# kouyt5/lightning-asr

Measured on AMD Instinct MI355X. Metric: audio-seconds/sec training (asr13x1, bs=32, 10 s clips), higher is better.
Workload: dtype bf16; 1 GPU; asr13x1 QuartzNet-CTC train step, bs=32/GPU, 10 s synthetic 16 kHz clips, labels.txt vocab (C=28), HIP mel+conv+CTC+NovoGrad, random-init weights; global_batch=32, n_class=28, parallelism=dp1, feature_prefetch=True, hip_graph=True, staged_backward=False

## Files before the change

lightning_asr_amd/csrc/conv.hip:

```cpp
#include "common.h"
#include "fused.h"

namespace lasr {

static thread_local const DwTapCtx* g_dw_tap_ctx = nullptr;
void dw_taps_set_ctx(const DwTapCtx* ctx) { g_dw_tap_ctx = ctx; }
bool dw_taps_enabled() {
  static const bool on = !(getenv("LASR_DW_TAPS") && atoi(getenv("LASR_DW_TAPS")) == 0);
  return on;
}
const uint32_t* dw_taps_for(const float* w, int flip, int64_t C) {
  (void)flip;
  const DwTapCtx* c = g_dw_tap_ctx;
  if (!c || C % 64 != 0) return nullptr;
  for (int i = 0; i < c->n; ++i)
    if (c->w[i] == w && c->C[i] == (int)C) return c->t[i];
  return nullptr;
}

static constexpr int kCB = 64;
static constexpr int kTT = 128;
static constexpr int kR = 8;
static constexpr int kMaxK = 128;

// ... 415 lines not shown
        o[0] += a[0]; o[1] += a[1]; o[2] += a[2]; o[3] += a[3];
      }
      Elem<bf16_t>::st4(y + off, o);
    }
  }
}

namespace dwm {
static constexpr int TT = 512;
static constexpr int KWMAX = 128;
static constexpr int TIN = TT - 16 + KWMAX;
static constexpr int LDI = 1296;
static constexpr int RS = 128;
static constexpr int LDST = 160;
static constexpr int IMG_BYTES = kCB * LDI;
static constexpr int STAGE_BYTES = RS * LDST;
static constexpr int WROW = 160;
static constexpr int WSM_OFF = IMG_BYTES + STAGE_BYTES;
static constexpr int SMEM = WSM_OFF + kCB * WROW * 4;
static_assert(LDI >= TIN * 2 && LDI % 16 == 0, "image pitch");
}
struct DwBnIn {
  const bf16_t* y; const bf16_t* y2; const float* coef; const float* coef2; bf16_t* out; int act;
};
typedef __bf16 dw_bf16x8 __attribute__((ext_vector_type(8)));
typedef float dw_f32x4 __attribute__((ext_vector_type(4)));
typedef short dw_s16x4 __attribute__((ext_vector_type(4)));

#ifdef LASR_DW_STAMPS
__device__ unsigned long long* g_dw_stamps = nullptr;
#define DW_STAMP(i_) do { if (g_dw_stamps && threadIdx.x == 0) g_dw_stamps[(blockIdx.y * gridDim.x + blockIdx.x) * 8 + (i_)] = wall_clock64(); } while (0)
#else
#define DW_STAMP(i_) do {} while (0)
#endif
template <int NKS, int NSET, bool FUSE = false>
__device__ __forceinline__ void dwconv_s1_mfma_body(const bf16_t* __restrict__ x, const float* __restrict__ w,
                                                    const bf16_t* __restrict__ addend, bf16_t* __restrict__ y,
                                                    int Tlen, int C, int k, int flip, int bx, int by, int bz, int gz,
                                                    char* smem_raw, const uint32_t* __restrict__ taps, const DwBnIn bn = DwBnIn{}) {
  using namespace dwm;
  char* img = smem_raw;
  char* stage = smem_raw + IMG_BYTES;
  uint32_t* wsm = reinterpret_cast<uint32_t*>(smem_raw + WSM_OFF);
  const int tid = threadIdx.x, lane = tid & 63, wid = tid >> 6;
  const int b = by, c0 = bx * kCB;
  if (taps) {
// ... 9 lines not shown
    float f0[kIt], f1[kIt];
#pragma unroll
    for (int it = 0; it < kIt; ++it) {
      const int i = tid + 512 * it;
      const int ch = i / WROW, idx = i - ch * WROW;
      const int i0 = idx < 80 ? 2 * idx : 2 * (idx - 80) + 1;
      const int j0 = i0 - 24, j1 = i0 - 23;
      const float* wc = w + (size_t)min(c0 + ch, C - 1) * k;
      const bool cok = c0 + ch < C;
      const int q0 = min(max(j0, 0), k - 1), q1 = min(max(j1, 0), k - 1);
      const float a0 = wc[flip ? k - 1 - q0 : q0], a1 = wc[flip ? k - 1 - q1 : q1];
      f0[it] = __uint_as_float(__float_as_uint(a0) & ((cok && j0 >= 0 && j0 < k) ? 0xffffffffu : 0u));
      f1[it] = __uint_as_float(__float_as_uint(a1) & ((cok && j1 >= 0 && j1 < k) ? 0xffffffffu : 0u));
    }
    __builtin_amdgcn_sched_barrier(0);
#pragma unroll
    for (int it = 0; it < kIt; ++it) wsm[tid + 512 * it] = (uint32_t)f32_to_bf16(f0[it]) | ((uint32_t)f32_to_bf16(f1[it]) << 16);
  }
  const int pad = k / 2, P = (pad + 7) & ~7, sh = P - pad;
  constexpr int KW = 32 * NKS;
  const bf16_t* xb = FUSE ? nullptr : x + (size_t)b * Tlen * C;
  const int n16 = lane & 15, g4 = lane >> 4;
  float ca[8], cb[8], ca2[8], cb2[8];
  if (FUSE) {
    const int ccl = min(c0 + ((tid & 7) << 3), C - 8);
    auto ld8 = [](const float* p, float (&o)[8]) {
      const float4 u = *reinterpret_cast<const float4*>(p), q = *reinterpret_cast<const float4*>(p + 4);
      o[0] = u.x; o[1] = u.y; o[2] = u.z; o[3] = u.w; o[4] = q.x; o[5] = q.y; o[6] = q.z; o[7] = q.w;
    };
    ld8(bn.coef + ccl, ca); ld8(bn.coef + C + ccl, cb);
    if (bn.y2) { ld8(bn.coef2 + ccl, ca2); ld8(bn.coef2 + C + ccl, cb2); }
  }

  DW_STAMP(0);
  constexpr int TTS = 256 * NSET;
  for (int tA = bz * TTS; tA < Tlen; tA += TTS * gz) {
    const int tin = TTS - 16 + KW;
    constexpr int kRounds = (TTS - 16 + KWMAX + RS - 1) / RS;
    uint4 v[kRounds][2];
    if (!FUSE) {
#pragma unroll
      for (int r = 0; r < kRounds; ++r) {
#pragma unroll
        for (int h = 0; h < 2; ++h) {
          const int ch = tid + 512 * h;
          const int tau = r * RS + (ch >> 3);
          const int t = tA - P + tau;
          const int cc = c0 + ((ch & 7) << 3);
          const bool ok = tau < tin && t >= 0 && t < Tlen && cc < C;
          const uint4 ld = *reinterpret_cast<const uint4*>(xb + (size_t)min(max(t, 0), Tlen - 1) * C + min(cc, C - 8));
          const uint32_t mk = ok ? 0xffffffffu : 0u;
          v[r][h] = make_uint4(ld.x & mk, ld.y & mk, ld.z & mk, ld.w & mk);
        }
      }
    } else {
      uint4 ly[kRounds][2], lr[kRounds][2];
      const size_t ub = (size_t)b * Tlen * C;
#pragma unroll
      for (int r = 0; r < kRounds; ++r) {
#pragma unroll
        for (int h = 0; h < 2; ++h) {
          const int ch = tid + 512 * h;
          const int t = tA - P + r * RS + (ch >> 3);
          const size_t off = ub + (size_t)min(max(t, 0), Tlen - 1) * C + min(c0 + ((ch & 7) << 3), C - 8);
          ly[r][h] = Vec<bf16_t>::raw(bn.y + off);
          if (bn.y2) lr[r][h] = Vec<bf16_t>::raw(bn.y2 + off);
        }
      }
      with_act(bn.act, [&](auto act_c) {
      constexpr int act = decltype(act_c)::value;
#pragma unroll
      for (int r = 0; r < kRounds; ++r) {
#pragma unroll
        for (int h = 0; h < 2; ++h) {
          const int ch = tid + 512 * h;
          const int tau = r * RS + (ch >> 3);
          const int t = tA - P + tau;
          const int cc = c0 + ((ch & 7) << 3);
          const bool ok = tau < tin && t >= 0 && t < Tlen && cc < C;
          float yv[8], rv[8], o[8];
          Vec<bf16_t>::unpack(ly[r][h], yv);
#pragma unroll
          for (int j = 0; j < 8; ++j) o[j] = fmaf(yv[j], ca[j], cb[j]);
          if (bn.y2) {
            Vec<bf16_t>::unpack(lr[r][h], rv);
#pragma unroll
            for (int j = 0; j < 8; ++j) o[j] += fmaf(rv[j], ca2[j], cb2[j]);
          }
#pragma unroll
          for (int j = 0; j < 8; ++j) o[j] = act_fwd(o[j], act);
          const uint4 pk = Vec<bf16_t>::pack(o);
// ... 822 lines not shown
        hipLaunchKernelGGL(dwconv_s1_bf16_kernel, grid, dim3(256), sh1, as_stream(stream), (const bf16_t*)x, w, (const bf16_t*)addend,
                           (bf16_t*)y, Tin, C, k, flip);
      }
    }
  } else {
    const bool small = (int64_t)grid.x * grid.y * grid.z < 200;
    const dim3 g2 = small ? dim3((unsigned)cdiv(Tout, 64), grid.y, grid.z) : grid;
#define LASR_DWF(T_, R_)                                                                                                          \
  do {                                                                                                                            \
    (void)hipFuncSetAttribute(reinterpret_cast<const void*>(dwconv_fwd_kernel<T_, R_>), hipFuncAttributeMaxDynamicSharedMemorySize, 160 * 1024); \
    hipLaunchKernelGGL((dwconv_fwd_kernel<T_, R_>), g2, dim3(256), shmem, as_stream(stream), (const T_*)x, w, (const T_*)addend, (T_*)y, Tin,  \
                       Tout, C, k, stride, flip);                                                                                 \
  } while (0)
    if (dtype == LASR_F32) { if (small) LASR_DWF(float, 4); else LASR_DWF(float, 8); }
    else { if (small) LASR_DWF(bf16_t, 4); else LASR_DWF(bf16_t, 8); }
#undef LASR_DWF
  }
  prof_end(tok, as_stream(stream));
  LASR_LAUNCH_CHECK("dwconv_fwd_kernel");
  return 0;
}

int lasr::dwconv_fwd_bn(const void* y, const float* coef, const void* y2, const float* coef2, int act, const float* w, void* out, void* u,
                        int64_t B, int64_t T, int64_t C, int k, void* stream) {
  LASR_CHECK_ARG(y && coef && w && out && u && (!y2 || coef2), "dwconv_fwd_bn: null pointer");
  static const bool off = getenv("LASR_DWCONV_FMA") || getenv("LASR_DWCONV_DOT2");
  const int padk = k / 2, shk = ((padk + 7) & ~7) - padk;
  auto al16 = [](const void* p) { return reinterpret_cast<uintptr_t>(p) % 16 == 0; };
  if (off || k < 1 || k > kMaxK || !(k & 1) || C % 8 != 0 || C < 8 || 15 + k + shk > dwm::KWMAX || T <= 0 || T >= (1 << 30) || B <= 0 ||
      B >= 65536 || !al16(y) || !al16(y2) || !al16(out) || !al16(u) || !al16(coef) || !al16(coef2))
    return 1;
  const int nks = (15 + k + shk + 31) / 32;
  static const bool no_half = getenv("LASR_DWCONV_NO_HALF") != nullptr;
  const bool half = !no_half && T > 256 && cdiv(C, kCB) * B * cdiv(T, (int64_t)512) < 200;
  static const bool full_too = getenv("LASR_BN_DW_FUSE") && atoi(getenv("LASR_BN_DW_FUSE")) == 2;
  if (!half && !full_too) return 1;
  const dim3 gridm((unsigned)cdiv(C, kCB), (unsigned)B, half ? (unsigned)std::min<int64_t>(cdiv(T, (int64_t)256), 8) : 1u);
  DwBnIn bn;
  bn.y = (const bf16_t*)y; bn.y2 = (const bf16_t*)y2; bn.coef = coef; bn.coef2 = coef2; bn.out = (bf16_t*)out; bn.act = act;
  const int tok = prof_begin(LASR_PROF_DWCONV, as_stream(stream), 2.0 * (double)B * T * C * k, (double)B * T * C * (y2 ? 4 : 3) * 2);
  const uint32_t* taps = dw_taps_for(w, 0, C);
#define LASR_DWMB2(N_, S_)                                                                                                  \
  do {                                                                                                                      \
    (void)hipFuncSetAttribute(reinterpret_cast<const void*>(dwconv_s1_mfma_bn_kernel<N_, S_>), hipFuncAttributeMaxDynamicSharedMemorySize, 160 * 1024); \
    hipLaunchKernelGGL((dwconv_s1_mfma_bn_kernel<N_, S_>), gridm, dim3(512), dwm::SMEM, as_stream(stream), bn, w, (bf16_t*)u, (int)T, (int)C, k, taps); \
  } while (0)
#define LASR_DWMB(N_) do { if (half) LASR_DWMB2(N_, 1); else LASR_DWMB2(N_, 2); } while (0)
  if (nks == 1) LASR_DWMB(1); else if (nks == 2) LASR_DWMB(2); else if (nks == 3) LASR_DWMB(3); else LASR_DWMB(4);
#undef LASR_DWMB
#undef LASR_DWMB2
  prof_end(tok, as_stream(stream));
  LASR_LAUNCH_CHECK("dwconv_s1_mfma_bn_kernel");
  return 0;
}

extern "C" size_t lasr_dwconv_wgrad_workspace_bytes(int64_t B, int64_t Tout, int64_t C, int k) {
  return (size_t)B * cdiv(Tout, kWChunkG) * C * k * sizeof(float);
}

static int dwconv_wgrad_impl(const void* x, const void* dy, float* dw, int dtype, int64_t B, int64_t Tin, int64_t C, int k,
                            int stride, void* workspace, size_t workspace_bytes, void* stream, int* n_partials_out);

// ... 170 lines not shown
```

lightning_asr_amd/csrc/fused.h:

```cpp
#pragma once
#include "common.h"

namespace lasr {

int dwconv_fwd_bn(const void* y, const float* coef, const void* y2, const float* coef2, int act, const float* w, void* out, void* u,
                  int64_t B, int64_t T, int64_t C, int k, void* stream);

static constexpr int kDwTapRow = 160;
struct DwTapJobs {
  int n; int blk0[17]; const float* w[16]; uint32_t* out[16]; int C[16]; int k[16];
};
__device__ __forceinline__ uint32_t dw_tap_entry(const float* __restrict__ w, int C, int k, int e) {
  const int flip = e / (C * kDwTapRow), r = e - flip * (C * kDwTapRow);
  const int c = r / kDwTapRow, idx = r - c * kDwTapRow;
  const int i0 = idx < kDwTapRow / 2 ? 2 * idx : 2 * (idx - kDwTapRow / 2) + 1;
  const int j0 = i0 - 24, j1 = i0 - 23;
  const float* wc = w + (size_t)c * k;
  const int q0 = min(max(j0, 0), k - 1), q1 = min(max(j1, 0), k - 1);
  const float a0 = wc[flip ? k - 1 - q0 : q0], a1 = wc[flip ? k - 1 - q1 : q1];
  const uint32_t m0 = (j0 >= 0 && j0 < k) ? 0xffffffffu : 0u, m1 = (j1 >= 0 && j1 < k) ? 0xffffffffu : 0u;
  return (uint32_t)f32_to_bf16(__uint_as_float(__float_as_uint(a0) & m0)) | ((uint32_t)f32_to_bf16(__uint_as_float(__float_as_uint(a1) & m1)) << 16);
}
struct DwTapCtx { int n; const float* w[16]; const uint32_t* t[16]; int C[16]; };
void dw_taps_set_ctx(const DwTapCtx* ctx);
const uint32_t* dw_taps_for(const float* w, int flip, int64_t C);
bool dw_taps_enabled();

int mask_lengths_step_cast(const float* pct, int64_t B, int64_t T_, int32_t* lens, uint64_t* step_counter, const float* in, void* out,
                           int64_t n, const DwTapJobs* jobs, void* stream);
// ... 12 lines not shown
```

lightning_asr_amd/csrc/model.hip:

```cpp
#include "common.h"
#include "mel.h"
#include "fused.h"
#include "gemm.h"
#include "lstm_body.h"
#include "se_seqsum.h"
#include <string>
#include <vector>
#include <math.h>

extern "C" size_t lasr_bn_bwd_workspace_bytes(int64_t B, int64_t T, int64_t C);
extern "C" size_t lasr_gemm_workspace_bytes(int64_t M, int64_t N, int split_k, int want_stats);
extern "C" size_t lasr_dwconv_wgrad_workspace_bytes(int64_t B, int64_t Tout, int64_t C, int k);
extern "C" int lasr_log_softmax_bwd(const float*, const float*, float*, int64_t, int64_t, void*);
extern "C" int lasr_cast_f32_to_bf16(const float*, void*, int64_t, void*);
extern "C" int lasr_colsum_f32(const float* x, float* out, int64_t rows, int64_t C, void* workspace, size_t workspace_bytes, void* stream);
extern "C" size_t lasr_colsum_workspace_bytes(int64_t rows, int64_t C);
extern "C" int lasr_scale_sum_f32(const float* x, int64_t n, float scale, float* out, void* stream);
extern "C" int lasr_seqsum(const void* x, int dtype, int64_t B, int64_t T, int64_t C, float* sums, void* stream);
extern "C" int lasr_se_fwd(const float* sums, const float* coef, const float* W1, const float* W2, int64_t B, int64_t T, int64_t C,
                           float* pooled, float* hidden, float* scale, void* stream);
extern "C" size_t lasr_se_bwd_workspace_bytes(int64_t B, int64_t C);
extern "C" int lasr_se_bwd(const void* dout, const void* y, const float* coef, const void* y2, const float* coef2, const float* scale,
                           const float* hidden, const float* pooled, const float* W1, const float* W2, int dtype, int64_t B, int64_t T,
                           int64_t C, int act, float* seg, float* dW1, float* dW2, void* workspace, size_t workspace_bytes, void* stream);
// ... 504 lines not shown
  if (!training) {
    std::vector<lasr_bn_eval_desc> descs;
    for (const Unit& u : m->units) {
      descs.push_back({params + u.bn.gamma, params + u.bn.beta, buffers + u.bn.rmean, buffers + u.bn.rvar, atf(ws, u.o_coef), u.co});
      if (u.has_res)
        descs.push_back({params + u.bn_res.gamma, params + u.bn_res.beta, buffers + u.bn_res.rmean, buffers + u.bn_res.rvar,
                         atf(ws, u.o_coef2), u.co});
    }
    for (size_t i = 0; i < descs.size(); i += 64)
      LASR_TRY(lasr_bn_eval_coef_many(descs.data() + i, (int)std::min<size_t>(64, descs.size() - i), kBnEps, stream));
    if (eval_fold(m->cfg.dtype)) {
      std::vector<lasr_fold_desc> fd;
      for (const Unit& u : m->units)
        if (fold_unit(u))
          fd.push_back({params + u.w_pw, params + u.w_res, atf(ws, u.o_coef), atf(ws, u.o_coef2), at(ws, u.o_wfold), atf(ws, u.o_bfold), u.co, u.ci});
      for (size_t i = 0; i < fd.size(); i += 32)
        LASR_TRY(lasr_fold_bn_weights_many(fd.data() + i, (int)std::min<size_t>(32, fd.size() - i), stream));
    }
  }
  const void* x = feats;
  int64_t Tx = T_in;
  static const bool bn_dw_fuse = !(getenv("LASR_BN_DW_FUSE") && atoi(getenv("LASR_BN_DW_FUSE")) == 0);
  const Unit* pend = nullptr;
  auto bn_act_of = [&](const Unit& v) -> int {
    ProfScope ps_bn(LASR_PROF_BN, stream, (double)N * v.co * dtype_size(dt) * (v.has_res ? 3 : 2));
    const lasr_dropout drop = {m->drop_step, m->drop_seed, (uint32_t)(&v - m->units.data()), dropping ? m->drop_p : 0.f};
    return lasr_bn_act_fwd_drop(at(ws, v.o_y), atf(ws, v.o_coef), v.has_res ? at(ws, v.o_y2) : nullptr,
                                v.has_res ? atf(ws, v.o_coef2) : nullptr, v.has_se ? atf(ws, v.o_se_scale) : nullptr, at(ws, v.o_out), dt, B,
                                T, v.co, v.act ? m->cfg.act : LASR_ACT_NONE, dropping ? &drop : nullptr, stream);
  };
  RoctxRange rr_fwd(training ? "lasr:forward (training)" : "lasr:forward (eval)");
  for (size_t ui = 0; ui < m->units.size(); ++ui) {
    const Unit& u = m->units[ui];
    RoctxRange rr_unit(u.rx_fwd.c_str());
    if (pend && !(u.has_dw && u.stride == 1 && !u.ctx_before)) {
      LASR_TRY(bn_act_of(*pend));
      pend = nullptr;
    }
    if (u.ctx_before) {
      {
        lasr_gemm_problem pr[2];
        for (int d = 0; d < 2; ++d) pr[d] = {x, wptr(m, params, ws, m->lstm.w_ih[d]), atf(ws, p.o_gx[d]), N, 160, 256, nullptr, nullptr, 0, nullptr};
        LASR_TRY(lasr_gemm_batch(pr, 2, dt, LASR_F32, 0, 0, 1, scratch, p.scratch_bytes, stream));
      }
      LASR_TRY(lasr_copy_cols(x, dt, 256, 0, at(ws, p.o_cat), dt, 336, 0, N, 256, 0, stream));
      LASR_TRY(lasr_bilstm_fwd(atf(ws, p.o_gx[0]), atf(ws, p.o_gx[1]), params + m->lstm.w_hh[0], params + m->lstm.w_hh[1],
                               params + m->lstm.b_ih[0], params + m->lstm.b_hh[0], params + m->lstm.b_ih[1], params + m->lstm.b_hh[1],
                               lens, B, T, at(ws, p.o_cat), dt, 336, 256, atf(ws, p.o_lstm_saved), stream));
      x = at(ws, p.o_cat);
    }
    const void* gin = x;
    if (u.has_dw) {
      int fused = 1;
      if (pend) {
        fused = dwconv_fwd_bn(at(ws, pend->o_y), atf(ws, pend->o_coef), pend->has_res ? at(ws, pend->o_y2) : nullptr,
                              pend->has_res ? atf(ws, pend->o_coef2) : nullptr, pend->act ? m->cfg.act : LASR_ACT_NONE, params + u.w_dw,
                              at(ws, pend->o_out), at(ws, u.o_u), B, T, u.ci, u.k, stream);
        if (fused < 0) return fused;
        if (fused == 1) LASR_TRY(bn_act_of(*pend));
        pend = nullptr;
      }
      if (fused == 1) LASR_TRY(lasr_dwconv_fwd(x, params + u.w_dw, nullptr, at(ws, u.o_u), dt, B, Tx, u.ci, u.k, u.stride, 0, stream));
      gin = at(ws, u.o_u);
    }
    if (!training && eval_fold(dt) && fold_unit(u)) {
      LASR_TRY(lasr_gemm_dual(gin, u.ci, x, u.ci, at(ws, u.o_wfold), atf(ws, u.o_bfold), at(ws, u.o_out), N, u.co, u.masked ? lens : nullptr,
                              T, u.act ? m->cfg.act : LASR_ACT_NONE, stream));
      x = at(ws, u.o_out);
      Tx = T;
      continue;
    }
    float* stats = training ? atf(ws, u.o_stats) : nullptr;
    float* stats2 = (training && u.has_res) ? atf(ws, u.o_stats2) : nullptr;
    bool se_sums_done = false;
    {
      lasr_gemm_problem pr[2];
      pr[0] = {gin, wptr(m, params, ws, u.w_pw), at(ws, u.o_y), N, u.co, u.ci, nullptr, u.masked ? lens : nullptr, T, stats};
      if (u.has_res) pr[1] = {x, wptr(m, params, ws, u.w_res), at(ws, u.o_y2), N, u.co, u.ci, nullptr, nullptr, 0, stats2};
      const int np = u.has_res ? 2 : 1;
      if (training && !no_fuse()) {
        const float* parts[2] = {nullptr, nullptr};
        int tiles[2] = {0, 0};
        LASR_TRY(lasr_gemm_batch_partials(pr, np, dt, dt, 0, 0, scratch, p.scratch_bytes, parts, tiles, stream));
        lasr_bn_branch br[2];
        br[0] = {parts[0], tiles[0], params + u.bn.gamma, params + u.bn.beta, buffers + u.bn.rmean, buffers + u.bn.rvar,
                 atf(ws, u.o_coef), atf(ws, u.o_saved), stats};
        if (u.has_res)
          br[1] = {parts[1], tiles[1], params + u.bn_res.gamma, params + u.bn_res.beta, buffers + u.bn_res.rmean,
                   buffers + u.bn_res.rvar, atf(ws, u.o_coef2), atf(ws, u.o_saved2), stats2};
        ProfScope ps(LASR_PROF_BN, stream, 0.0);
        int merged = 1;
        if (u.has_se) {
          merged = bn_finalize_partials_seqsum(br, np, u.co, N, kBnEps, kBnMom, at(ws, u.o_y), dt, B, T, atf(ws, u.o_se_sum), stream);
          if (merged < 0 || merged > 1) return merged;
          se_sums_done = merged == 0;
        }
        if (merged == 1) LASR_TRY(lasr_bn_finalize_partials(br, np, u.co, N, kBnEps, kBnMom, stream));
      } else {
        LASR_TRY(lasr_gemm_batch(pr, np, dt, dt, 0, 0, 1, scratch, p.scratch_bytes, stream));
        if (training) {
          LASR_TRY(lasr_bn_finalize(stats, params + u.bn.gamma, params + u.bn.beta, buffers + u.bn.rmean, buffers + u.bn.rvar,
                                    atf(ws, u.o_coef), atf(ws, u.o_saved), u.co, N, kBnEps, kBnMom, training, stream));
          if (u.has_res)
            LASR_TRY(lasr_bn_finalize(stats2, params + u.bn_res.gamma, params + u.bn_res.beta, buffers + u.bn_res.rmean,
                                      buffers + u.bn_res.rvar, atf(ws, u.o_coef2), atf(ws, u.o_saved2), u.co, N, kBnEps, kBnMom,
                                      training, stream));
        }
      }
    }
    bool se_applied = false;
    if (u.has_se) {
      ProfScope ps_se(LASR_PROF_BN, stream, (double)N * u.co * dtype_size(dt));
      if (!se_sums_done) LASR_TRY(lasr_seqsum(at(ws, u.o_y), dt, B, T, u.co, atf(ws, u.o_se_sum), stream));
      int folded = 1;
      if (training && !dropping && !no_fuse())
        folded = bn_se_act_fwd(at(ws, u.o_y), atf(ws, u.o_coef), u.has_res ? at(ws, u.o_y2) : nullptr, u.has_res ? atf(ws, u.o_coef2) : nullptr,
                               atf(ws, u.o_se_sum), params + u.w_se1, params + u.w_se2, at(ws, u.o_out), atf(ws, u.o_se_pool),
                               atf(ws, u.o_se_hid), atf(ws, u.o_se_scale), dt, B, T, u.co, u.act ? m->cfg.act : LASR_ACT_NONE, stream);
      if (folded < 0 || folded > 1) return folded;
      se_applied = folded == 0;
// ... 387 lines not shown
```

lightning_asr_amd/csrc/norm.hip:

```cpp
#include "common.h"
#include "reduce_body.h"
#include "se_seqsum.h"
#include "fused.h"
#include "dropout.h"
#include <algorithm>
#include <string.h>

namespace lasr {

template <typename T, bool TO_BTC>
__global__ __launch_bounds__(256) void transpose_kernel(const void* __restrict__ in_, void* __restrict__ out_,
                                                        int64_t C, int64_t Tt) {
  __shared__ float tile[32][33];
  const int b = blockIdx.z;
  const int64_t c0 = (int64_t)blockIdx.y * 32, t0 = (int64_t)blockIdx.x * 32;
  const int tx = threadIdx.x & 31, ty = threadIdx.x >> 5;
  if (TO_BTC) {
    const float* in = reinterpret_cast<const float*>(in_) + (int64_t)b * C * Tt;
    T* out = reinterpret_cast<T*>(out_) + (int64_t)b * C * Tt;
    for (int i = ty; i < 32; i += 8)
      if (c0 + i < C && t0 + tx < Tt) tile[i][tx] = in[(c0 + i) * Tt + t0 + tx];
    __syncthreads();
    for (int i = ty; i < 32; i += 8)
      if (t0 + i < Tt && c0 + tx < C) Elem<T>::st(out + (t0 + i) * C + c0 + tx, tile[tx][i]);
  } else {
    const T* in = reinterpret_cast<const T*>(in_) + (int64_t)b * C * Tt;
    float* out = reinterpret_cast<float*>(out_) + (int64_t)b * C * Tt;
// ... 21 lines not shown
    return;
  }
  if ((int)blockIdx.x >= cast_blocks) {
    const int tb = (int)blockIdx.x - cast_blocks;
    int l = 0;
    while (l + 1 < jobs.n && jobs.blk0[l + 1] <= tb) ++l;
    const int e = (tb - jobs.blk0[l]) * 256 + (int)threadIdx.x;
    if (e < 2 * jobs.C[l] * kDwTapRow) jobs.out[l][e] = dw_tap_entry(jobs.w[l], jobs.C[l], jobs.k[l], e);
    return;
  }
  const int64_t n4 = n >> 2;
  const int64_t stride = (int64_t)cast_blocks * 256;
  for (int64_t e = blockIdx.x * (int64_t)256 + threadIdx.x; e < n4; e += stride) {
    const float4 v = reinterpret_cast<const float4*>(in)[e];
    uint2 o;
    o.x = (uint32_t)f32_to_bf16(v.x) | ((uint32_t)f32_to_bf16(v.y) << 16);
    o.y = (uint32_t)f32_to_bf16(v.z) | ((uint32_t)f32_to_bf16(v.w) << 16);
    reinterpret_cast<uint2*>(out)[e] = o;
  }
  if (blockIdx.x == 0)
    for (int64_t e = (n4 << 2) + threadIdx.x; e < n; e += 256) out[e] = f32_to_bf16(in[e]);
}

__device__ __forceinline__ void bn_finalize_channel(float s, float q, int64_t c, const float* __restrict__ gamma,
                                                    const float* __restrict__ beta, float* __restrict__ rmean,
                                                    float* __restrict__ rvar, float* __restrict__ coef, float* __restrict__ saved,
                                                    int64_t C, float n, float eps, float momentum, int training) {
  float mean, var;
  if (training) {
    const double m = (double)s / n;
    double v = (double)q / n - m * m;
    if (v < 0) v = 0;
    mean = (float)m;
    var = (float)v;
    if (rmean) {
      rmean[c] = (1.f - momentum) * rmean[c] + momentum * mean;
      const float unbiased = n > 1.f ? (float)(v * (double)n / ((double)n - 1.0)) : var;
      rvar[c] = (1.f - momentum) * rvar[c] + momentum * unbiased;
    }
  } else {
    mean = rmean[c];
    var = rvar[c];
  }
  const float rstd = 1.0f / sqrtf(var + eps);
  const float a = gamma[c] * rstd;
  coef[c] = a;
  coef[C + c] = beta[c] - mean * a;
  if (saved) { saved[c] = mean; saved[C + c] = rstd; }
}

__global__ void bn_finalize_kernel(const float* __restrict__ stats, const float* __restrict__ gamma,
                                   const float* __restrict__ beta, float* __restrict__ rmean, float* __restrict__ rvar,
                                   float* __restrict__ coef, float* __restrict__ saved, int64_t C, float n, float eps,
                                   float momentum, int training) {
  const int64_t c = blockIdx.x * (int64_t)blockDim.x + threadIdx.x;
  if (c >= C) return;
  bn_finalize_channel(training ? stats[c] : 0.f, training ? stats[C + c] : 0.f, c, gamma, beta, rmean, rvar, coef, saved, C, n, eps,
                      momentum, training);
}

struct BnEvalMany { lasr_bn_eval_desc d[64]; };
__global__ __launch_bounds__(256) void bn_eval_coef_many_kernel(BnEvalMany a, float eps) {
  const lasr_bn_eval_desc q = a.d[blockIdx.y];
  const int64_t c = blockIdx.x * (int64_t)blockDim.x + threadIdx.x;
  if (c >= q.C) return;
  bn_finalize_channel(0.f, 0.f, c, q.gamma, q.beta, const_cast<float*>(q.running_mean), const_cast<float*>(q.running_var), q.coef, nullptr,
                      q.C, 1.f, eps, 0.f, 0);
}

template <int LANES = 8>
__device__ __forceinline__ double partial_lane_sum(const float* __restrict__ partials, int n_part, int64_t ncols, int64_t c, int pl) {
  double a0 = 0.0, a1 = 0.0, a2 = 0.0, a3 = 0.0;
  for (int p = pl; p < n_part; p += 16 * LANES) {
    float v[16];
#pragma unroll
    for (int i = 0; i < 16; ++i) {
      const int r = p + LANES * i;
      const float x = partials[(int64_t)min(r, n_part - 1) * ncols + c];
      v[i] = r < n_part ? x : 0.f;
    }
#pragma unroll
    for (int i = 0; i < 16; i += 4) {
      a0 += (double)v[i]; a1 += (double)v[i + 1]; a2 += (double)v[i + 2]; a3 += (double)v[i + 3];
    }
  }
  return (a0 + a1) + (a2 + a3);
}

__global__ __launch_bounds__(256) void reduce_partials_kernel(const float* __restrict__ partials, int n_part, int64_t ncols,
                                                              float* __restrict__ out0, int64_t split, float* __restrict__ out1) {
  __shared__ double s_acc[8][33];
  const int cl = threadIdx.x & 31, pl = threadIdx.x >> 5;
  const int64_t c = (int64_t)blockIdx.x * 32 + cl;
  s_acc[pl][cl] = c < ncols ? partial_lane_sum(partials, n_part, ncols, c, pl) : 0.0;
  __syncthreads();
  if (pl == 0 && c < ncols) {
    double s = 0.0;
#pragma unroll
    for (int i = 0; i < 8; ++i) s += s_acc[i][cl];
    if (c < split) out0[c] = (float)s;
    else if (out1) out1[c - split] = (float)s;
  }
}

struct BnBranch {
  const float* partials; int n_part;
  const float* gamma; const float* beta; float* rmean; float* rvar; float* coef; float* saved; float* stats;
};
struct BnBranch2 { BnBranch b[2]; };

__global__ __launch_bounds__(256) void bn_finalize_partials_kernel(BnBranch2 br, int64_t C, float n, float eps, float momentum) {
  __shared__ double s_acc[8][33];
  const BnBranch& b = blockIdx.y ? br.b[1] : br.b[0];
  const int cl = threadIdx.x & 31, pl = threadIdx.x >> 5;
  const int64_t c = (int64_t)blockIdx.x * 16 + (cl & 15);
  s_acc[pl][cl] = c < C ? partial_lane_sum(b.partials, b.n_part, 2 * C, (int64_t)(cl >> 4) * C + c, pl) : 0.0;
  __syncthreads();
  if (pl == 0 && cl < 16 && c < C) {
    double s = 0.0, q = 0.0;
#pragma unroll
    for (int i = 0; i < 8; ++i) { s += s_acc[i][cl]; q += s_acc[i][16 + cl]; }
    if (b.stats) { b.stats[c] = (float)s; b.stats[C + c] = (float)q; }
    bn_finalize_channel((float)s, (float)q, c, b.gamma, b.beta, b.rmean, b.rvar, b.coef, b.saved, C, n, eps, momentum, 1);
  }
}

template <typename T>
__global__ __launch_bounds__(256) void bn_finalize_seqsum_kernel(BnBranch2 br, int64_t C, float n, float eps, float momentum, int nfx, int nf,
                                                                 const T* __restrict__ x, int Tt, int gx, float* __restrict__ sums) {
  constexpr int RL = 256 / (64 / Vec<T>::kN);
  __shared__ double s_acc[8][33];
  __shared__ float s_red[RL][65];
// ... 147 lines not shown
      for (int j = 0; j < V; ++j) {
        o[j] = fmaf(v[j], a[j], b[j]);
        if (SE) o[j] *= sev[u][j];
      }
      float dsc[V];
      if (DROP) drop_scale<V>(drop, drop_step, off[u], dsc);
      if (DROP && HAS2) {
#pragma unroll
        for (int j = 0; j < V; ++j) o[j] *= dsc[j];
      }
      if (HAS2) {
        Vec<T>::unpack(rw[u], w);
        tab_vec(s_tab + 2 * C, c, C, a); tab_vec(s_tab + 3 * C, c, C, b);
#pragma unroll
        for (int j = 0; j < V; ++j) o[j] += fmaf(w[j], a[j], b[j]);
      }
#pragma unroll
      for (int j = 0; j < V; ++j) o[j] = act_fwd(o[j], act);
      if (DROP && !HAS2) {
#pragma unroll
        for (int j = 0; j < V; ++j) o[j] *= dsc[j];
      }
      if (it0 + 256 * u < n_items) Vec<T>::store(out + off[u], o);
    }
  }
  });
}

template <typename T, bool HAS2, bool SE, bool DROP>
__global__ __launch_bounds__(256, 2) void bn_bwd_stats_kernel(const T* __restrict__ dout, const T* __restrict__ y,
                                                              const float* __restrict__ coef, const float* __restrict__ saved,
                                                              const T* __restrict__ y2, const float* __restrict__ coef2,
                                                              const float* __restrict__ saved2, const float* __restrict__ se,
                                                              const float* __restrict__ seg, float* __restrict__ partials,
                                                              int rows, int Tt, int C, int act, DropArgs drop, int per_utt) {
  extern __shared__ __attribute__((aligned(16))) float s_part[];
  constexpr int V = Vec<T>::kN;
  const unsigned long long drop_step = DROP ? *drop.step : 0ull;
  constexpr int RB = 2;
  const ColGeom g = col_geom<V>(C);
  int r0 = blockIdx.x * kRowsPerBlock;
  int r1 = min(r0 + kRowsPerBlock, rows);
  if (per_utt) {
    const int nslab = (Tt + kRowsPerBlock - 1) / kRowsPerBlock;
    const int ub = blockIdx.x / nslab, sl = blockIdx.x - ub * nslab;
    r0 = ub * Tt + sl * kRowsPerBlock;
// ... 549 lines not shown
  const size_t shmem = (size_t)4 * C * sizeof(float);
  if (y2) {
    if (se_scale) { DISPATCH_DTYPE(dtype, { if (da.step) { hipLaunchKernelGGL((bn_act_fwd_kernel<T, true, true, true>), dim3((unsigned)cdiv(rows, kFwdSlabRows)), dim3(256), shmem,
                                             as_stream(stream), (const T*)y, coef, (const T*)y2, coef2, se_scale, (T*)out, (int)rows,
                                             (int)T_, (int)C, act, da); } else { hipLaunchKernelGGL((bn_act_fwd_kernel<T, true, true, false>), dim3((unsigned)cdiv(rows, kFwdSlabRows)), dim3(256), shmem,
                                             as_stream(stream), (const T*)y, coef, (const T*)y2, coef2, se_scale, (T*)out, (int)rows,
                                             (int)T_, (int)C, act, da); } }); } else { DISPATCH_DTYPE(dtype, { if (da.step) { hipLaunchKernelGGL((bn_act_fwd_kernel<T, true, false, true>), dim3((unsigned)cdiv(rows, kFwdSlabRows)), dim3(256), shmem,
                                             as_stream(stream), (const T*)y, coef, (const T*)y2, coef2, se_scale, (T*)out, (int)rows,
                                             (int)T_, (int)C, act, da); } else { hipLaunchKernelGGL((bn_act_fwd_kernel<T, true, false, false>), dim3((unsigned)cdiv(rows, kFwdSlabRows)), dim3(256), shmem,
                                             as_stream(stream), (const T*)y, coef, (const T*)y2, coef2, se_scale, (T*)out, (int)rows,
                                             (int)T_, (int)C, act, da); } }); }
  } else {
    if (se_scale) { DISPATCH_DTYPE(dtype, { if (da.step) { hipLaunchKernelGGL((bn_act_fwd_kernel<T, false, true, true>), dim3((unsigned)cdiv(rows, kFwdSlabRows)), dim3(256), shmem,
                                             as_stream(stream), (const T*)y, coef, (const T*)y2, coef2, se_scale, (T*)out, (int)rows,
                                             (int)T_, (int)C, act, da); } else { hipLaunchKernelGGL((bn_act_fwd_kernel<T, false, true, false>), dim3((unsigned)cdiv(rows, kFwdSlabRows)), dim3(256), shmem,
                                             as_stream(stream), (const T*)y, coef, (const T*)y2, coef2, se_scale, (T*)out, (int)rows,
                                             (int)T_, (int)C, act, da); } }); } else { DISPATCH_DTYPE(dtype, { if (da.step) { hipLaunchKernelGGL((bn_act_fwd_kernel<T, false, false, true>), dim3((unsigned)cdiv(rows, kFwdSlabRows)), dim3(256), shmem,
                                             as_stream(stream), (const T*)y, coef, (const T*)y2, coef2, se_scale, (T*)out, (int)rows,
                                             (int)T_, (int)C, act, da); } else { hipLaunchKernelGGL((bn_act_fwd_kernel<T, false, false, false>), dim3((unsigned)cdiv(rows, kFwdSlabRows)), dim3(256), shmem,
                                             as_stream(stream), (const T*)y, coef, (const T*)y2, coef2, se_scale, (T*)out, (int)rows,
                                             (int)T_, (int)C, act, da); } }); }
  }
  LASR_LAUNCH_CHECK("bn_act_fwd_kernel");
  return 0;
}

extern "C" int lasr_bn_act_fwd(const void* y, const float* coef, const void* y2, const float* coef2, const float* se_scale,
                               void* out, int dtype, int64_t B, int64_t T_, int64_t C, int act, void* stream) {
  return lasr_bn_act_fwd_drop(y, coef, y2, coef2, se_scale, out, dtype, B, T_, C, act, nullptr, stream);
}

extern "C" size_t lasr_bn_bwd_workspace_bytes(int64_t B, int64_t T_, int64_t C) {
  return (size_t)cdiv(B * T_, kRowsPerBlock) * 4 * C * sizeof(float) + (size_t)10 * C * sizeof(float);
}

extern "C" int lasr_bn_act_bwd_stats(const void* dout, const void* y, const float* coef, const float* saved, const void* y2,
                                     const float* coef2, const float* saved2, const float* se_scale, const float* se_grad,
                                     float* sums, float* sums2, int dtype, int64_t B, int64_t T_, int64_t C, int act,
                                     void* workspace, size_t workspace_bytes, void* stream) {
  return lasr_bn_act_bwd_stats_drop(dout, y, coef, saved, y2, coef2, saved2, se_scale, se_grad, sums, sums2, dtype, B, T_, C, act, nullptr,
                                    workspace, workspace_bytes, stream);
}

extern "C" int lasr_bn_act_bwd_stats_drop(const void* dout, const void* y, const float* coef, const float* saved, const void* y2,
                                          const float* coef2, const float* saved2, const float* se_scale, const float* se_grad,
                                          float* sums, float* sums2, int dtype, int64_t B, int64_t T_, int64_t C, int act,
// ... 431 lines not shown
```

Measured before the change: 161,000 audio-seconds/sec.

## Fold BN partial-stat finalization into the consuming BN-act and dwconv kernels

Drops the separate BN finalize kernel after each pointwise GEMM and defers it. Each consumer (the fused depthwise conv or a new slab BN-act kernel) reduces the partials per 64-channel slab in LDS, computes the coefficients locally, and only the first row-block writes running stats and saved values. The aim is fewer launches and less serialization between GEMM and consumer. The cost is that every workgroup redundantly re-reduces the partials, and it adds shared-memory use and a new code path with an owed-finalize state machine.

Result: faster. 162,900 audio-seconds/sec (median of 6 runs) (+1.2%).

```diff
diff --git a/lightning_asr_amd/csrc/bn_fin.h b/lightning_asr_amd/csrc/bn_fin.h
--- /dev/null
+++ b/lightning_asr_amd/csrc/bn_fin.h
@@ -0,0 +1,121 @@
+#pragma once
+#include "common.h"
+
+namespace lasr {
+
+__device__ __forceinline__ void bn_finalize_channel(float s, float q, int64_t c, const float* __restrict__ gamma,
+                                                    const float* __restrict__ beta, float* __restrict__ rmean,
+                                                    float* __restrict__ rvar, float* __restrict__ coef, float* __restrict__ saved,
+                                                    int64_t C, float n, float eps, float momentum, int training,
+                                                    float* sa = nullptr, float* sb = nullptr) {
+  float mean, var;
+  if (training) {
+    const double m = (double)s / n;
+    double v = (double)q / n - m * m;
+    if (v < 0) v = 0;
+    mean = (float)m;
+    var = (float)v;
+    if (rmean) {
+      rmean[c] = (1.f - momentum) * rmean[c] + momentum * mean;
+      const float unbiased = n > 1.f ? (float)(v * (double)n / ((double)n - 1.0)) : var;
+      rvar[c] = (1.f - momentum) * rvar[c] + momentum * unbiased;
+    }
+  } else {
+    mean = rmean[c];
+    var = rvar[c];
+  }
+  const float rstd = 1.0f / sqrtf(var + eps);
+  const float a = gamma[c] * rstd;
+  const float b = beta[c] - mean * a;
+  if (coef) { coef[c] = a; coef[C + c] = b; }
+  if (saved) { saved[c] = mean; saved[C + c] = rstd; }
+  if (sa) { *sa = a; *sb = b; }
+}
+
+template <int LANES = 8>
+__device__ __forceinline__ double partial_lane_sum(const float* __restrict__ partials, int n_part, int64_t ncols, int64_t c, int pl) {
+  double a0 = 0.0, a1 = 0.0, a2 = 0.0, a3 = 0.0;
+  for (int p = pl; p < n_part; p += 16 * LANES) {
+    float v[16];
+#pragma unroll
+    for (int i = 0; i < 16; ++i) {
+      const int r = p + LANES * i;
+      const float x = partials[(int64_t)min(r, n_part - 1) * ncols + c];
+      v[i] = r < n_part ? x : 0.f;
+    }
+#pragma unroll
+    for (int i = 0; i < 16; i += 4) {
+      a0 += (double)v[i]; a1 += (double)v[i + 1]; a2 += (double)v[i + 2]; a3 += (double)v[i + 3];
+    }
+  }
+  return (a0 + a1) + (a2 + a3);
+}
+
+__device__ __forceinline__ void partial_lane_sum4(const float* __restrict__ partials, int n_part, int64_t ncols, int64_t c, int pl,
+                                                  double (&out)[4]) {
+  constexpr int LANES = 8;
+  double a0[4] = {0.0, 0.0, 0.0, 0.0}, a1[4] = {0.0, 0.0, 0.0, 0.0}, a2[4] = {0.0, 0.0, 0.0, 0.0}, a3[4] = {0.0, 0.0, 0.0, 0.0};
+  for (int p = pl; p < n_part; p += 8 * LANES) {
+    float4 v[8];
+#pragma unroll
+    for (int i = 0; i < 8; ++i) {
+      const int r = p + LANES * i;
+      const float4 x = *reinterpret_cast<const float4*>(partials + (int64_t)min(r, n_part - 1) * ncols + c);
+      const bool ok = r < n_part;
+      v[i] = make_float4(ok ? x.x : 0.f, ok ? x.y : 0.f, ok ? x.z : 0.f, ok ? x.w : 0.f);
+    }
+#pragma unroll
+    for (int i = 0; i < 8; i += 4) {
+      a0[0] += (double)v[i].x; a1[0] += (double)v[i + 1].x; a2[0] += (double)v[i + 2].x; a3[0] += (double)v[i + 3].x;
+      a0[1] += (double)v[i].y; a1[1] += (double)v[i + 1].y; a2[1] += (double)v[i + 2].y; a3[1] += (double)v[i + 3].y;
+      a0[2] += (double)v[i].z; a1[2] += (double)v[i + 1].z; a2[2] += (double)v[i + 2].z; a3[2] += (double)v[i + 3].z;
+      a0[3] += (double)v[i].w; a1[3] += (double)v[i + 1].w; a2[3] += (double)v[i + 2].w; a3[3] += (double)v[i + 3].w;
+    }
+  }
+#pragma unroll
+  for (int j = 0; j < 4; ++j) out[j] = (a0[j] + a1[j]) + (a2[j] + a3[j]);
+}
+
+struct BnBranch {
+  const float* partials; int n_part;
+  const float* gamma; const float* beta; float* rmean; float* rvar; float* coef; float* saved; float* stats;
+};
+struct BnBranch2 { BnBranch b[2]; };
+
+static constexpr int kBnSlabCh = 64;
+static constexpr int kBnSlabAccBytes = 8 * 2 * 2 * kBnSlabCh * 8;
+static constexpr int kBnSlabLdsBytes = kBnSlabAccBytes + 2 * 2 * kBnSlabCh * 4;
+
+__device__ __forceinline__ void bn_slab_finalize(const BnBranch2& br, int nbr, int C, int c0, float n, float eps, float momentum, bool side,
+                                                 char* lds) {
+  double* s_acc = reinterpret_cast<double*>(lds);
+  float* s_coef = reinterpret_cast<float*>(lds + kBnSlabAccBytes);
+  const int tid = threadIdx.x, bi = tid >> 8, pl = (tid >> 5) & 7, q = tid & 31;
+  const int cc = c0 + 4 * (q & 15);
+  if (bi < nbr && cc < C) {
+    const BnBranch& b = bi ? br.b[1] : br.b[0];
+    double s[4];
+    partial_lane_sum4(b.partials, b.n_part, 2 * (int64_t)C, (int64_t)(q >> 4) * C + cc, pl, s);
+    *reinterpret_cast<double2*>(s_acc + pl * 256 + bi * 128 + 4 * q) = make_double2(s[0], s[1]);
+    *reinterpret_cast<double2*>(s_acc + pl * 256 + bi * 128 + 4 * q + 2) = make_double2(s[2], s[3]);
+  }
+  __syncthreads();
+  if (tid < 2 * kBnSlabCh) {
+    const int fb = tid >> 6, ch = tid & 63, c = c0 + ch;
+    float a = 0.f, sh = 0.f;
+    if (fb < nbr && c < C) {
+      const BnBranch& b = fb ? br.b[1] : br.b[0];
+      double s = 0.0, qq = 0.0;
+#pragma unroll
+      for (int i = 0; i < 8; ++i) { s += s_acc[i * 256 + fb * 128 + ch]; qq += s_acc[i * 256 + fb * 128 + 64 + ch]; }
+      if (side && b.stats) { b.stats[c] = (float)s; b.stats[C + c] = (float)qq; }
+      bn_finalize_channel((float)s, (float)qq, c, b.gamma, b.beta, side ? b.rmean : nullptr, side ? b.rvar : nullptr, side ? b.coef : nullptr,
+                          side ? b.saved : nullptr, C, n, eps, momentum, 1, &a, &sh);
+    }
+    s_coef[fb * 128 + ch] = a;
+    s_coef[fb * 128 + 64 + ch] = sh;
+  }
+  __syncthreads();
+}
+
+}
diff --git a/lightning_asr_amd/csrc/conv.hip b/lightning_asr_amd/csrc/conv.hip
--- a/lightning_asr_amd/csrc/conv.hip
+++ b/lightning_asr_amd/csrc/conv.hip
@@ -1,5 +1,6 @@
 #include "common.h"
 #include "fused.h"
+#include "bn_fin.h"
 
 namespace lasr {
 
@@ -461,6 +462,7 @@
 }
 struct DwBnIn {
   const bf16_t* y; const bf16_t* y2; const float* coef; const float* coef2; bf16_t* out; int act;
+  BnBranch2 fin; int nbr; float n, eps, momentum;
 };
 typedef __bf16 dw_bf16x8 __attribute__((ext_vector_type(8)));
 typedef float dw_f32x4 __attribute__((ext_vector_type(4)));
@@ -516,7 +518,8 @@
   const bf16_t* xb = FUSE ? nullptr : x + (size_t)b * Tlen * C;
   const int n16 = lane & 15, g4 = lane >> 4;
   float ca[8], cb[8], ca2[8], cb2[8];
-  if (FUSE) {
+  bool fin_owed = FUSE && bn.nbr > 0;
+  if (FUSE && !fin_owed) {
     const int ccl = min(c0 + ((tid & 7) << 3), C - 8);
     auto ld8 = [](const float* p, float (&o)[8]) {
       const float4 u = *reinterpret_cast<const float4*>(p), q = *reinterpret_cast<const float4*>(p + 4);
@@ -525,6 +528,19 @@
     ld8(bn.coef + ccl, ca); ld8(bn.coef + C + ccl, cb);
     if (bn.y2) { ld8(bn.coef2 + ccl, ca2); ld8(bn.coef2 + C + ccl, cb2); }
   }
+
+  auto fin_slab = [&]() {
+    bn_slab_finalize(bn.fin, bn.nbr, C, c0, bn.n, bn.eps, bn.momentum, by == 0 && bz == 0, smem_raw);
+    const float* s_coef = reinterpret_cast<const float*>(smem_raw + kBnSlabAccBytes);
+    const int o = min(c0 + ((tid & 7) << 3), C - 8) - c0;
+    auto ld8 = [](const float* p, float (&v)[8]) {
+      const float4 u = *reinterpret_cast<const float4*>(p), q = *reinterpret_cast<const float4*>(p + 4);
+      v[0] = u.x; v[1] = u.y; v[2] = u.z; v[3] = u.w; v[4] = q.x; v[5] = q.y; v[6] = q.z; v[7] = q.w;
+    };
+    ld8(s_coef + o, ca); ld8(s_coef + kBnSlabCh + o, cb);
+    if (bn.y2) { ld8(s_coef + 2 * kBnSlabCh + o, ca2); ld8(s_coef + 3 * kBnSlabCh + o, cb2); }
+  };
+  if (NSET == 2 && fin_owed) { fin_slab(); fin_owed = false; }
 
   DW_STAMP(0);
   constexpr int TTS = 256 * NSET;
@@ -561,6 +577,7 @@
           if (bn.y2) lr[r][h] = Vec<bf16_t>::raw(bn.y2 + off);
         }
       }
+      if (NSET == 1 && fin_owed) { fin_slab(); fin_owed = false; }
       with_act(bn.act, [&](auto act_c) {
       constexpr int act = decltype(act_c)::value;
 #pragma unroll
@@ -1429,8 +1446,9 @@
 }
 
 int lasr::dwconv_fwd_bn(const void* y, const float* coef, const void* y2, const float* coef2, int act, const float* w, void* out, void* u,
-                        int64_t B, int64_t T, int64_t C, int k, void* stream) {
-  LASR_CHECK_ARG(y && coef && w && out && u && (!y2 || coef2), "dwconv_fwd_bn: null pointer");
+                        int64_t B, int64_t T, int64_t C, int k, void* stream, const BnFinDesc* fin) {
+  LASR_CHECK_ARG(y && w && out && u && (fin || (coef && (!y2 || coef2))), "dwconv_fwd_bn: null pointer");
+  if (fin) { coef = fin->br[0].coef; coef2 = y2 ? fin->br[1].coef : nullptr; }
   static const bool off = getenv("LASR_DWCONV_FMA") || getenv("LASR_DWCONV_DOT2");
   const int padk = k / 2, shk = ((padk + 7) & ~7) - padk;
   auto al16 = [](const void* p) { return reinterpret_cast<uintptr_t>(p) % 16 == 0; };
@@ -1445,6 +1463,12 @@
   const dim3 gridm((unsigned)cdiv(C, kCB), (unsigned)B, half ? (unsigned)std::min<int64_t>(cdiv(T, (int64_t)256), 8) : 1u);
   DwBnIn bn;
   bn.y = (const bf16_t*)y; bn.y2 = (const bf16_t*)y2; bn.coef = coef; bn.coef2 = coef2; bn.out = (bf16_t*)out; bn.act = act;
+  bn.nbr = 0; bn.n = bn.eps = bn.momentum = 0.f;
+  if (fin) {
+    LASR_CHECK_ARG(fin->nbr == (y2 ? 2 : 1), "dwconv_fwd_bn: branch count");
+    LASR_TRY(bn_branches_of(fin, &bn.fin));
+    bn.nbr = fin->nbr; bn.n = (float)fin->n_rows; bn.eps = fin->eps; bn.momentum = fin->momentum;
+  }
   const int tok = prof_begin(LASR_PROF_DWCONV, as_stream(stream), 2.0 * (double)B * T * C * k, (double)B * T * C * (y2 ? 4 : 3) * 2);
   const uint32_t* taps = dw_taps_for(w, 0, C);
 #define LASR_DWMB2(N_, S_)                                                                                                  \
diff --git a/lightning_asr_amd/csrc/fused.h b/lightning_asr_amd/csrc/fused.h
--- a/lightning_asr_amd/csrc/fused.h
+++ b/lightning_asr_amd/csrc/fused.h
@@ -1,10 +1,26 @@
 #pragma once
 #include "common.h"
+#include "bn_fin.h"
 
 namespace lasr {
 
+struct BnFinDesc {
+  lasr_bn_branch br[2]; int nbr; int64_t n_rows; float eps, momentum;
+};
 int dwconv_fwd_bn(const void* y, const float* coef, const void* y2, const float* coef2, int act, const float* w, void* out, void* u,
-                  int64_t B, int64_t T, int64_t C, int k, void* stream);
+                  int64_t B, int64_t T, int64_t C, int k, void* stream, const BnFinDesc* fin = nullptr);
+inline int bn_branches_of(const BnFinDesc* f, BnBranch2* out) {
+  LASR_CHECK_ARG(f->nbr == 1 || f->nbr == 2, "bn finalize: bad branch count");
+  for (int i = 0; i < 2; ++i) {
+    const lasr_bn_branch& q = f->br[i < f->nbr ? i : 0];
+    LASR_CHECK_ARG(q.partials && q.n_partials > 0 && q.gamma && q.beta && q.coef && reinterpret_cast<uintptr_t>(q.partials) % 16 == 0,
+                   "bn finalize: null or misaligned pointer");
+    out->b[i] = {q.partials, q.n_partials, q.gamma, q.beta, q.running_mean, q.running_var, q.coef, q.saved, q.stats};
+  }
+  return 0;
+}
+int bn_act_fwd_fin(const BnFinDesc* fin, const void* y, const void* y2, void* out, int dtype, int64_t B, int64_t T_, int64_t C, int act,
+                   void* stream);
 
 static constexpr int kDwTapRow = 160;
 struct DwTapJobs {
diff --git a/lightning_asr_amd/csrc/model.hip b/lightning_asr_amd/csrc/model.hip
--- a/lightning_asr_amd/csrc/model.hip
+++ b/lightning_asr_amd/csrc/model.hip
@@ -550,8 +550,18 @@
   int64_t Tx = T_in;
   static const bool bn_dw_fuse = !(getenv("LASR_BN_DW_FUSE") && atoi(getenv("LASR_BN_DW_FUSE")) == 0);
   const Unit* pend = nullptr;
+  static const bool fin_consumer = !(getenv("LASR_BN_FIN_CONSUMER") && atoi(getenv("LASR_BN_FIN_CONSUMER")) == 0);
+  BnFinDesc owed;
+  const Unit* owed_by = nullptr;
   auto bn_act_of = [&](const Unit& v) -> int {
     ProfScope ps_bn(LASR_PROF_BN, stream, (double)N * v.co * dtype_size(dt) * (v.has_res ? 3 : 2));
+    if (owed_by == &v) {
+      owed_by = nullptr;
+      const int r = bn_act_fwd_fin(&owed, at(ws, v.o_y), v.has_res ? at(ws, v.o_y2) : nullptr, at(ws, v.o_out), dt, B, T, v.co,
+                                   v.act ? m->cfg.act : LASR_ACT_NONE, stream);
+      if (r != 1) return r;
+      LASR_TRY(lasr_bn_finalize_partials(owed.br, owed.nbr, v.co, owed.n_rows, owed.eps, owed.momentum, stream));
+    }
     const lasr_dropout drop = {m->drop_step, m->drop_seed, (uint32_t)(&v - m->units.data()), dropping ? m->drop_p : 0.f};
     return lasr_bn_act_fwd_drop(at(ws, v.o_y), atf(ws, v.o_coef), v.has_res ? at(ws, v.o_y2) : nullptr,
                                 v.has_res ? atf(ws, v.o_coef2) : nullptr, v.has_se ? atf(ws, v.o_se_scale) : nullptr, at(ws, v.o_out), dt, B,
@@ -583,8 +593,9 @@
       if (pend) {
         fused = dwconv_fwd_bn(at(ws, pend->o_y), atf(ws, pend->o_coef), pend->has_res ? at(ws, pend->o_y2) : nullptr,
                               pend->has_res ? atf(ws, pend->o_coef2) : nullptr, pend->act ? m->cfg.act : LASR_ACT_NONE, params + u.w_dw,
-                              at(ws, pend->o_out), at(ws, u.o_u), B, T, u.ci, u.k, stream);
+                              at(ws, pend->o_out), at(ws, u.o_u), B, T, u.ci, u.k, stream, owed_by == pend ? &owed : nullptr);
         if (fused < 0) return fused;
+        if (fused == 0 && owed_by == pend) owed_by = nullptr;
         if (fused == 1) LASR_TRY(bn_act_of(*pend));
         pend = nullptr;
       }
@@ -606,6 +617,7 @@
       pr[0] = {gin, wptr(m, params, ws, u.w_pw), at(ws, u.o_y), N, u.co, u.ci, nullptr, u.masked ? lens : nullptr, T, stats};
       if (u.has_res) pr[1] = {x, wptr(m, params, ws, u.w_res), at(ws, u.o_y2), N, u.co, u.ci, nullptr, nullptr, 0, stats2};
       const int np = u.has_res ? 2 : 1;
+      LASR_CHECK_ARG(!owed_by, "lasr forward: a BN finalize is still owed when the next GEMM overwrites its partials");
       if (training && !no_fuse()) {
         const float* parts[2] = {nullptr, nullptr};
         int tiles[2] = {0, 0};
@@ -616,14 +628,21 @@
         if (u.has_res)
           br[1] = {parts[1], tiles[1], params + u.bn_res.gamma, params + u.bn_res.beta, buffers + u.bn_res.rmean,
                    buffers + u.bn_res.rvar, atf(ws, u.o_coef2), atf(ws, u.o_saved2), stats2};
-        ProfScope ps(LASR_PROF_BN, stream, 0.0);
-        int merged = 1;
-        if (u.has_se) {
-          merged = bn_finalize_partials_seqsum(br, np, u.co, N, kBnEps, kBnMom, at(ws, u.o_y), dt, B, T, atf(ws, u.o_se_sum), stream);
-          if (merged < 0 || merged > 1) return merged;
-          se_sums_done = merged == 0;
+        if (fin_consumer && dt == LASR_BF16 && !u.has_se && !dropping) {
+          owed.br[0] = br[0];
+          if (u.has_res) owed.br[1] = br[1];
+          owed.nbr = np; owed.n_rows = N; owed.eps = kBnEps; owed.momentum = kBnMom;
+          owed_by = &u;
+        } else {
+          ProfScope ps(LASR_PROF_BN, stream, 0.0);
+          int merged = 1;
+          if (u.has_se) {
+            merged = bn_finalize_partials_seqsum(br, np, u.co, N, kBnEps, kBnMom, at(ws, u.o_y), dt, B, T, atf(ws, u.o_se_sum), stream);
+            if (merged < 0 || merged > 1) return merged;
+            se_sums_done = merged == 0;
+          }
+          if (merged == 1) LASR_TRY(lasr_bn_finalize_partials(br, np, u.co, N, kBnEps, kBnMom, stream));
         }
-        if (merged == 1) LASR_TRY(lasr_bn_finalize_partials(br, np, u.co, N, kBnEps, kBnMom, stream));
       } else {
         LASR_TRY(lasr_gemm_batch(pr, np, dt, dt, 0, 0, 1, scratch, p.scratch_bytes, stream));
         if (training) {
diff --git a/lightning_asr_amd/csrc/norm.hip b/lightning_asr_amd/csrc/norm.hip
--- a/lightning_asr_amd/csrc/norm.hip
+++ b/lightning_asr_amd/csrc/norm.hip
@@ -3,6 +3,7 @@
 #include "se_seqsum.h"
 #include "fused.h"
 #include "dropout.h"
+#include "bn_fin.h"
 #include <algorithm>
 #include <string.h>
 
@@ -70,33 +71,6 @@
     for (int64_t e = (n4 << 2) + threadIdx.x; e < n; e += 256) out[e] = f32_to_bf16(in[e]);
 }
 
-__device__ __forceinline__ void bn_finalize_channel(float s, float q, int64_t c, const float* __restrict__ gamma,
-                                                    const float* __restrict__ beta, float* __restrict__ rmean,
-                                                    float* __restrict__ rvar, float* __restrict__ coef, float* __restrict__ saved,
-                                                    int64_t C, float n, float eps, float momentum, int training) {
-  float mean, var;
-  if (training) {
-    const double m = (double)s / n;
-    double v = (double)q / n - m * m;
-    if (v < 0) v = 0;
-    mean = (float)m;
-    var = (float)v;
-    if (rmean) {
-      rmean[c] = (1.f - momentum) * rmean[c] + momentum * mean;
-      const float unbiased = n > 1.f ? (float)(v * (double)n / ((double)n - 1.0)) : var;
-      rvar[c] = (1.f - momentum) * rvar[c] + momentum * unbiased;
-    }
-  } else {
-    mean = rmean[c];
-    var = rvar[c];
-  }
-  const float rstd = 1.0f / sqrtf(var + eps);
-  const float a = gamma[c] * rstd;
-  coef[c] = a;
-  coef[C + c] = beta[c] - mean * a;
-  if (saved) { saved[c] = mean; saved[C + c] = rstd; }
-}
-
 __global__ void bn_finalize_kernel(const float* __restrict__ stats, const float* __restrict__ gamma,
                                    const float* __restrict__ beta, float* __restrict__ rmean, float* __restrict__ rvar,
                                    float* __restrict__ coef, float* __restrict__ saved, int64_t C, float n, float eps,
@@ -114,25 +88,6 @@
   if (c >= q.C) return;
   bn_finalize_channel(0.f, 0.f, c, q.gamma, q.beta, const_cast<float*>(q.running_mean), const_cast<float*>(q.running_var), q.coef, nullptr,
                       q.C, 1.f, eps, 0.f, 0);
-}
-
-template <int LANES = 8>
-__device__ __forceinline__ double partial_lane_sum(const float* __restrict__ partials, int n_part, int64_t ncols, int64_t c, int pl) {
-  double a0 = 0.0, a1 = 0.0, a2 = 0.0, a3 = 0.0;
-  for (int p = pl; p < n_part; p += 16 * LANES) {
-    float v[16];
-#pragma unroll
-    for (int i = 0; i < 16; ++i) {
-      const int r = p + LANES * i;
-      const float x = partials[(int64_t)min(r, n_part - 1) * ncols + c];
-      v[i] = r < n_part ? x : 0.f;
-    }
-#pragma unroll
-    for (int i = 0; i < 16; i += 4) {
-      a0 += (double)v[i]; a1 += (double)v[i + 1]; a2 += (double)v[i + 2]; a3 += (double)v[i + 3];
-    }
-  }
-  return (a0 + a1) + (a2 + a3);
 }
 
 __global__ __launch_bounds__(256) void reduce_partials_kernel(const float* __restrict__ partials, int n_part, int64_t ncols,
@@ -151,11 +106,6 @@
   }
 }
 
-struct BnBranch {
-  const float* partials; int n_part;
-  const float* gamma; const float* beta; float* rmean; float* rvar; float* coef; float* saved; float* stats;
-};
-struct BnBranch2 { BnBranch b[2]; };
 
 __global__ __launch_bounds__(256) void bn_finalize_partials_kernel(BnBranch2 br, int64_t C, float n, float eps, float momentum) {
   __shared__ double s_acc[8][33];
@@ -349,6 +299,62 @@
         for (int j = 0; j < V; ++j) o[j] *= dsc[j];
       }
       if (it0 + 256 * u < n_items) Vec<T>::store(out + off[u], o);
+    }
+  }
+  });
+}
+
+static constexpr int kFinRows = 4;
+static constexpr int kFinTargetWgs = 256;
+template <bool HAS2>
+__global__ __launch_bounds__(512) void bn_act_fwd_slab_kernel(BnBranch2 br, const bf16_t* __restrict__ y, const bf16_t* __restrict__ y2,
+                                                              bf16_t* __restrict__ out, int rows, int C, int rpc, int act_rt, float n,
+                                                              float eps, float momentum) {
+  __shared__ __attribute__((aligned(16))) char lds[kBnSlabLdsBytes];
+  const int tid = threadIdx.x, oc = tid & 7, rl = tid >> 3;
+  const int c0 = blockIdx.x * kBnSlabCh;
+  const bool cok = c0 + oc * 8 < C;
+  const int cc = min(c0 + oc * 8, C - 8);
+  const int r0 = blockIdx.y * rpc, r1 = min(r0 + rpc, rows);
+  uint4 ly[kFinRows], lr[kFinRows];
+  auto issue = [&](int rb) {
+#pragma unroll
+    for (int u = 0; u < kFinRows; ++u) {
+      const uint32_t off = (uint32_t)min(rb + 64 * u, r1 - 1) * (uint32_t)C + (uint32_t)cc;
+      ly[u] = Vec<bf16_t>::raw(y + off);
+      if (HAS2) lr[u] = Vec<bf16_t>::raw(y2 + off);
+    }
+  };
+  issue(r0 + rl);
+  bn_slab_finalize(br, HAS2 ? 2 : 1, C, c0, n, eps, momentum, blockIdx.y == 0, lds);
+  float a[8], b[8], a2[8], b2[8];
+  {
+    const float* s_coef = reinterpret_cast<const float*>(lds + kBnSlabAccBytes) + (cc - c0);
+    lds_vec8(s_coef, a); lds_vec8(s_coef + kBnSlabCh, b);
+    if (HAS2) { lds_vec8(s_coef + 2 * kBnSlabCh, a2); lds_vec8(s_coef + 3 * kBnSlabCh, b2); }
+  }
+  with_act(act_rt, [&](auto act_c) {
+  constexpr int act = decltype(act_c)::value;
+  for (int rb = r0 + rl; rb < r1; rb += 64 * kFinRows) {
+    uint4 cy[kFinRows], cr[kFinRows];
+#pragma unroll
+    for (int u = 0; u < kFinRows; ++u) { cy[u] = ly[u]; if (HAS2) cr[u] = lr[u]; }
+    if (rb + 64 * kFinRows < r1) issue(rb + 64 * kFinRows);
+#pragma unroll
+    for (int u = 0; u < kFinRows; ++u) {
+      float v[8], o[8];
+      Vec<bf16_t>::unpack(cy[u], v);
+#pragma unroll
+      for (int j = 0; j < 8; ++j) o[j] = fmaf(v[j], a[j], b[j]);
+      if (HAS2) {
+        Vec<bf16_t>::unpack(cr[u], v);
+#pragma unroll
+        for (int j = 0; j < 8; ++j) o[j] += fmaf(v[j], a2[j], b2[j]);
+      }
+#pragma unroll
+      for (int j = 0; j < 8; ++j) o[j] = act_fwd(o[j], act);
+      const int row = rb + 64 * u;
+      if (cok && row < r1) Vec<bf16_t>::store(out + (uint32_t)row * (uint32_t)C + (uint32_t)cc, o);
     }
   }
   });
@@ -944,6 +950,29 @@
                                              (int)T_, (int)C, act, da); } }); }
   }
   LASR_LAUNCH_CHECK("bn_act_fwd_kernel");
+  return 0;
+}
+
+int lasr::bn_act_fwd_fin(const BnFinDesc* fin, const void* y, const void* y2, void* out, int dtype, int64_t B, int64_t T_, int64_t C, int act,
+                   void* stream) {
+  auto al16 = [](const void* p) { return reinterpret_cast<uintptr_t>(p) % 16 == 0; };
+  if (dtype != LASR_BF16 || C % 8 != 0 || C > 4096 || B <= 0 || T_ <= 0 || B * T_ * C >= ((int64_t)1 << 31) || !al16(y) || !al16(y2) ||
+      !al16(out))
+    return 1;
+  LASR_CHECK_ARG(fin && y && out && fin->nbr == (y2 ? 2 : 1), "bn_act_fwd_fin: bad argument");
+  BnBranch2 br;
+  LASR_TRY(bn_branches_of(fin, &br));
+  const int64_t rows = B * T_, nslab = cdiv(C, (int64_t)kBnSlabCh);
+  const int64_t nchunk0 = std::max<int64_t>(1, kFinTargetWgs / nslab);
+  const int64_t rpc = cdiv(cdiv(rows, nchunk0), (int64_t)64) * 64;
+  const dim3 grid((unsigned)nslab, (unsigned)cdiv(rows, rpc));
+  if (y2)
+    hipLaunchKernelGGL(bn_act_fwd_slab_kernel<true>, grid, dim3(512), 0, as_stream(stream), br, (const bf16_t*)y, (const bf16_t*)y2,
+                       (bf16_t*)out, (int)rows, (int)C, (int)rpc, act, (float)fin->n_rows, fin->eps, fin->momentum);
+  else
+    hipLaunchKernelGGL(bn_act_fwd_slab_kernel<false>, grid, dim3(512), 0, as_stream(stream), br, (const bf16_t*)y, nullptr, (bf16_t*)out,
+                       (int)rows, (int)C, (int)rpc, act, (float)fin->n_rows, fin->eps, fin->momentum);
+  LASR_LAUNCH_CHECK("bn_act_fwd_slab_kernel");
   return 0;
 }
 
```
